# VinAIResearch/GaPro

Measured on AMD Instinct MI355X. Metric: scenes/sec pseudo-label gen (ScanNetV2-train-shaped synthetic scenes), higher is better.
Workload: dtype f64

## Files before the change

### gapro_amd/csrc/svgp_fit.hip

```cpp
#include <math.h>

#include <algorithm>
#include <type_traits>
#include <vector>

#include "common.h"
#include "fit_layout.h"
#include "fit_math.h"
#include "epilogue.h"
#ifdef GAPRO_DEBUG_TU
#include "../../include/gapro_hip_debug.h"
#include "mfma64.h"
#endif

namespace {
using namespace gapro_fit;

#ifndef GAPRO_NT
#define GAPRO_NT 512
#endif
constexpr int NT = GAPRO_NT;
constexpr int NW = NT / 64;
constexpr int kMaxMpLds = 512;
constexpr int kMaxDynLds = 150 * 1024;
// ... 353 lines not shown
                                     const gd* __restrict__ Q, int ld, const gd* __restrict__ qscale, KRange kr,
                                     Epi epi, ldsd* ring) {
  static_assert(NT == 512 || !sizeof(Epi), "gemm_wg: eight waves, one k row of a chunk per wave");
  static_assert(PF == 2 || PF == 4, "gemm_wg: register stages");
  rows16 = uni(rows16);
  cols16 = uni(cols16);
  lower_only = uni((int)lower_only) != 0;
  ld = uni(ld);
  P = uni_ptr(P);
  Q = uni_ptr(Q);
  qscale = uni_ptr(qscale);
  const int wave = uni(threadIdx.x >> 6), lane = threadIdx.x & 63, lr = lane & 15, lq = lane >> 4;
  const int rows = 16 * rows16, cols = 16 * cols16;
  const int nti = (rows + kWgTile - 1) / kWgTile, ntj = (cols + kWgTile - 1) / kWgTile;
  const int wi = wave < 4 ? wave : 7 - wave, wj = wave >> 2;
  const int kmax = TRIM ? uni((g_sh.f.M + 7) / 8 * 8) : ld;
  const int lcol = 2 * lane;
  const int lds_wr = wave * kWgRow + lcol;
  const int fa = lq * kWgRow + 32 * wi + lr;
  const int fb = kWgKC * kWgRow + lq * kWgRow + 64 * wj + lr;
#pragma nounroll
  for (int ti = 0; ti < nti; ++ti) {
#pragma nounroll
    for (int tj = 0; tj < (lower_only ? ti + 1 : ntj); ++tj) {
      const int I0 = kWgTile * ti, J0 = kWgTile * tj;
      int klo = 1 << 30, khi = 0, plo = 1 << 30, phi = 0;
      unsigned on_mask = 0;
      if (rows - I0 >= kWgTile && cols - J0 >= kWgTile) {
        int lo, hi, d;
        kr(I0, J0, &lo, &d);
        kr(I0 + kWgTile - 16, J0 + kWgTile - 16, &d, &hi);
        hi = hi < kmax ? hi : kmax;
        if (lo < hi) { klo = lo; khi = hi; }
        const int pi0 = I0 + 32 * wi, pj0 = J0 + 64 * wj;
#pragma unroll
        for (int u = 0; u < 2; ++u)
#pragma unroll
          for (int v = 0; v < 4; ++v)
            if (!(lower_only && pi0 + 16 * u < pj0 + 16 * v)) on_mask |= 1u << (4 * u + v);
        if (on_mask) {
          kr(pi0, pj0, &lo, &d);
          kr(pi0 + 16, pj0 + 48, &d, &hi);
          hi = hi < kmax ? hi : kmax;
          if (lo < hi) { plo = lo; phi = hi; }
        }
      } else {
#pragma nounroll
        for (int bi = 0; bi < kWgTile / 16; ++bi) {
          const int ib = I0 + 16 * bi;
          if (ib >= rows) break;
#pragma nounroll
          for (int bj = 0; bj < kWgTile / 16; ++bj) {
            const int jb = J0 + 16 * bj;
            if (jb >= cols) break;
            if (lower_only && ib < jb) continue;
            const bool mine = (bi >> 1) == wi && (bj >> 2) == wj;
            if (mine) on_mask |= 1u << (4 * (bi & 1) + (bj & 3));
            int lo, hi;
            kr(ib, jb, &lo, &hi);
            hi = hi < kmax ? hi : kmax;
            if (lo >= hi) continue;
            klo = lo < klo ? lo : klo;
            khi = hi > khi ? hi : khi;
            if (mine) {
              plo = lo < plo ? lo : plo;
              phi = hi > phi ? hi : phi;
            }
          }
        }
      }
      klo = uni(klo) & ~(kWgKC - 1);
      khi = uni(khi);
      plo = uni(plo) & ~(kWgKC - 1);
      phi = uni(phi);
      on_mask = (unsigned)uni((int)on_mask);
      const int nch = klo < khi ? (khi - klo + kWgKC - 1) / kWgKC : 0;
      d4 acc[2][4];
#pragma unroll
      for (int u = 0; u < 2; ++u)
#pragma unroll
        for (int v = 0; v < 4; ++v) acc[u][v] = (d4){0.0, 0.0, 0.0, 0.0};
      if (nch > 0) {
        const bool pin = I0 + lcol < ld, qin = J0 + lcol < ld;
        const gd* pg = P + (size_t)wave * ld + (pin ? I0 + lcol : 0);
        const gd* qg = Q + (size_t)wave * ld + (qin ? J0 + lcol : 0);
        d2 rp[PF], rq[PF];
        double rs[PF];
        auto gload = [&](int n, d2& p, d2& q, double& sc) {
          n = n < nch ? n : nch - 1;
          const size_t o = (size_t)(klo + kWgKC * n) * ld;
          p = *(const g_d2*)(pg + o);
          q = *(const g_d2*)(qg + o);
          if (SCALE) sc = qscale[klo + kWgKC * n + wave];
        };
        auto lstore = [&](int stage, const d2& p, const d2& q, double sc) {
          ldsd* base = ring + stage * kWgStage + lds_wr;
          *(lds_d2*)base = p;
          *(lds_d2*)(base + kWgKC * kWgRow) = SCALE ? (d2){q[0] * sc, q[1] * sc} : q;
        };
        double fa0[2], fb0[4], fa1[2], fb1[4];
        auto rd = [&](int stage, int s, double (&a)[2], double (&b)[4]) {
          const ldsd* st = ring + stage * kWgStage + 4 * s * kWgRow;
#pragma unroll
          for (int v = 0; v < 4; ++v) b[v] = st[fb + 16 * v];
#pragma unroll
          for (int u = 0; u < 2; ++u) a[u] = st[fa + 16 * u];
        };
        auto mm = [&](int k0, const double (&a)[2], const double (&b)[4]) {
          if (k0 < plo || k0 >= phi) return;
#pragma unroll
          for (int u = 0; u < 2; ++u)
#pragma unroll
            for (int v = 0; v < 4; ++v)
              acc[u][v] = __builtin_amdgcn_mfma_f64_16x16x4f64(a[u], b[v], acc[u][v], 0, 0, 0);
        };
        auto chunk = [&](auto cur_tag, auto slot_tag, int c) {
          constexpr int CUR = decltype(cur_tag)::value, SLOT = decltype(slot_tag)::value;
          const int k0 = klo + kWgKC * c;
          lstore(CUR ^ 1, rp[SLOT], rq[SLOT], rs[SLOT]);
          gload(c + 1 + PF, rp[SLOT], rq[SLOT], rs[SLOT]);
          rd(CUR, 1, fa1, fb1);
          __builtin_amdgcn_sched_barrier(0);
          mm(k0, fa0, fb0);
          __builtin_amdgcn_sched_barrier(0);
          __syncthreads();
          rd(CUR ^ 1, 0, fa0, fb0);
          __builtin_amdgcn_sched_barrier(0);
          mm(k0, fa1, fb1);
          __builtin_amdgcn_sched_barrier(0);
        };
        using I0t = std::integral_constant<int, 0>;
        using I1t = std::integral_constant<int, 1>;
        using I2t = std::integral_constant<int, 2>;
        using I3t = std::integral_constant<int, 3>;
#pragma unroll
        for (int n = 0; n < PF; ++n) gload(n, rp[n], rq[n], rs[n]);
        lstore(0, rp[0], rq[0], rs[0]);
        gload(PF, rp[0], rq[0], rs[0]);
        __syncthreads();
        rd(0, 0, fa0, fb0);
        int c = 0;
        if constexpr (PF == 2) {
#pragma nounroll
          for (; c + 1 < nch; c += 2) {
            chunk(I0t{}, I1t{}, c);
            chunk(I1t{}, I0t{}, c + 1);
          }
          if (c < nch) chunk(I0t{}, I1t{}, c);
        } else {
#pragma nounroll
          for (; c + 3 < nch; c += 4) {
            chunk(I0t{}, I1t{}, c);
            chunk(I1t{}, I2t{}, c + 1);
            chunk(I0t{}, I3t{}, c + 2);
            chunk(I1t{}, I0t{}, c + 3);
          }
          if (c < nch) chunk(I0t{}, I1t{}, c);
          if (c + 1 < nch) chunk(I1t{}, I2t{}, c + 1);
          if (c + 2 < nch) chunk(I0t{}, I3t{}, c + 2);
        }
      }
      run_epilogue<8>(epi,
                      [&](int b, int* i, int* j) {
                        const bool on = (on_mask >> b) & 1u;
                        *i = on ? I0 + 32 * wi + 16 * (b >> 2) : -1;
                        *j = J0 + 64 * wj + 16 * (b & 3);
                      },
                      [&](int b) -> const d4& { return acc[b >> 2][b & 3]; });
    }
  }
}

__device__ inline void store_tile(const d4& v, gd* __restrict__ Cm, gd* __restrict__ CT, int ld, int i0, int j0,
                                  ldsd* tile ) {
  const int lane = threadIdx.x & 63, lr = lane & 15, lq = lane >> 4;
  if (Cm) {
#pragma unroll
    for (int r = 0; r < 4; ++r) Cm[(size_t)(i0 + lq + 4 * r) * ld + j0 + lr] = v[r];
  }
  if (CT) {
#pragma unroll
    for (int r = 0; r < 4; ++r) tile[(lq + 4 * r) * 17 + lr] = v[r];
    __builtin_amdgcn_fence(__ATOMIC_RELEASE, "wavefront", "local");
    __builtin_amdgcn_wave_barrier();
#pragma unroll
    for (int r = 0; r < 4; ++r) CT[(size_t)(j0 + lq + 4 * r) * ld + i0 + lr] = tile[lr * 17 + lq + 4 * r];
    __builtin_amdgcn_fence(__ATOMIC_ACQUIRE, "wavefront", "local");
    __builtin_amdgcn_wave_barrier();
  }
}

__device__ __noinline__ void diag_factor_invert(ldsd* panel, int kb) {
  const Fit& f = g_sh.f;
  const int Mp = f.Mp;
  kb = uni(kb);
  gd* LT = f.mat[B_LT];
  const int lane = threadIdx.x & 63, r = lane & 15;
#ifdef GAPRO_PROFILE
  const unsigned long long tp0 = wall_clock64();
#endif
  double rdiag[16];
  {
    double a[16];
#pragma unroll
    for (int c = 0; c < 16; ++c) a[c] = panel[r * 17 + c];
    bool bad = false;
#pragma unroll
    for (int j = 0; j < 16; ++j) {
      double d = lane_bcast(a[j], j);
      if (!(d > 0.0)) {
        bad = true;
        d = 1e-30;
      }
      const double rs = rsqrt(d);
      rdiag[j] = rs;
      const double lj = (r == j) ? d * rs : a[j] * rs;
      a[j] = lj;
#pragma unroll
      for (int c = j + 1; c < 16; ++c) a[c] -= lj * lane_bcast(lj, c);
    }
    if (bad && lane == 0) g_sh.chol_bad = 1;
    if (lane < 16) {
#pragma unroll
      for (int c = 0; c < 16; ++c) g_sh.dblk[r * 17 + c] = (c <= r) ? a[c] : 0.0;
    }
  }
  __builtin_amdgcn_fence(__ATOMIC_SEQ_CST, "wavefront", "local");
  __builtin_amdgcn_wave_barrier();
#ifdef GAPRO_PROFILE
  const unsigned long long tp1 = wall_clock64();
#endif
  {
    double x[16], b[16];
#pragma unroll
    for (int rr = 0; rr < 16; ++rr) b[rr] = (rr == r) ? 1.0 : 0.0;
#pragma unroll
    for (int q = 0; q < 16; ++q) {
      x[q] = (q >= r) ? b[q] * rdiag[q] : 0.0;
#pragma unroll
      for (int rr = q + 1; rr < 16; ++rr) b[rr] = fma(-g_sh.dblk[rr * 17 + q], x[q], b[rr]);
    }
    if (lane < 16) {
#pragma unroll
      for (int c = 0; c < 16; ++c) g_sh.dinv[c * 17 + r] = x[c];
    }
  }
  __builtin_amdgcn_fence(__ATOMIC_SEQ_CST, "wavefront", "local");
  __builtin_amdgcn_wave_barrier();
#ifdef GAPRO_PROFILE
  const unsigned long long tp2 = wall_clock64();
#endif
#pragma unroll
  for (int e = 0; e < 4; ++e) {
    const int idx = lane + 64 * e;
    const int rr = idx >> 4, cc = idx & 15;
    LT[(size_t)(16 * kb + rr) * Mp + 16 * kb + cc] = g_sh.dblk[cc * 17 + rr];
    f.dinv[(size_t)kb * 256 + idx] = g_sh.dinv[rr * 17 + cc];
    f.dinvT[(size_t)kb * 256 + idx] = g_sh.dinv[cc * 17 + rr];
  }
#ifdef GAPRO_PROFILE
  if (lane == 0) {
    const unsigned long long tp3 = wall_clock64();
    g_sh.prof[22] += tp1 - tp0;
    g_sh.prof[23] += tp2 - tp1;
    g_sh.prof[24] += tp3 - tp2;
  }
#endif
}

__device__ inline void chol_update_tile(d4& acc, const gd* pa, const gd* pb, int Mp, int Q) {
  const size_t st = (size_t)4 * Mp;
  auto ld = [&](int q, double (&a)[4], double (&b)[4]) {
    const size_t o = (size_t)q * Mp;
#pragma unroll
    for (int e = 0; e < 4; ++e) {
      a[e] = pa[o + e * st];
      b[e] = pb[o + e * st];
    }
  };
  auto mm = [&](double (&a)[4], double (&b)[4]) {
#pragma unroll
    for (int e = 0; e < 4; ++e) acc = __builtin_amdgcn_mfma_f64_16x16x4f64(-a[e], b[e], acc, 0, 0, 0);
  };
  if (Q <= 0) return;
  double a0[4], b0[4], a1[4], b1[4];
  ld(0, a0, b0);
  int q = 0;
#pragma nounroll
  for (; q + 32 < Q; q += 32) {
    ld(q + 16, a1, b1);
    mm(a0, b0);
    ld(q + 32, a0, b0);
    mm(a1, b1);
  }
  if (q + 16 < Q) {
    ld(q + 16, a1, b1);
    mm(a0, b0);
    mm(a1, b1);
  } else {
    mm(a0, b0);
  }
}

template <int DC>
__device__ __noinline__ void cholesky_fused(const ldsd* Zt, ldsd* panel, double s, double inv_l2, double jitter) {
  const Fit& f = g_sh.f;
  Shared& sh = g_sh;
  const int Mp = f.Mp, M = f.M, D = DC ? DC : f.D, nb = Mp / 16;
  gd* LT = f.mat[B_LT];
  const int wave = __builtin_amdgcn_readfirstlane(threadIdx.x >> 6), lane = threadIdx.x & 63;
  const int lr = lane & 15, lq = lane >> 4;
  for (int kb = 0; kb < nb; ++kb) {
    for (int ib = kb + wave; ib < nb; ib += NW) {
      d4 acc;
      const int col = 16 * kb + lr;
#pragma unroll
      for (int r = 0; r < 4; ++r) {
        const int row = 16 * ib + lq + 4 * r;
        double v = 0.0;
        if (row < M && col < M) {
          v = s * gapro_fit_math::rbf_exp(-0.5 * inv_l2 * sqdist_t(Zt, row, Zt, col, D, Mp));
          if (row == col) v += jitter;
        } else if (row == col) {
          v = 1.0;
        }
        acc[r] = v;
      }
      const gd* pa = LT + (size_t)lq * Mp + 16 * ib + lr;
      const gd* pb = LT + (size_t)lq * Mp + 16 * kb + lr;
      chol_update_tile(acc, pa, pb, Mp, 16 * kb);
      ldsd* dst = panel + (16 * (ib - kb)) * 17;
#pragma unroll
      for (int r = 0; r < 4; ++r) dst[(lq + 4 * r) * 17 + lr] = acc[r];
    }
    __syncthreads();
    prof_stamp(0);
    if (wave == 0) diag_factor_invert(panel, kb);
    __syncthreads();
    prof_stamp(5);
    const int rows_below = Mp - 16 * (kb + 1);
    ldsd* pb = panel + 16 * 17;
    for (int idx = threadIdx.x; idx < rows_below * 16; idx += NT) {
      const int i = idx >> 4, c = idx & 15;
      double acc = 0.0;
#pragma unroll
      for (int q = 0; q < 16; ++q) acc += (q <= c) ? pb[i * 17 + q] * sh.dinv[c * 17 + q] : 0.0;
      __builtin_amdgcn_fence(__ATOMIC_SEQ_CST, "wavefront", "local");
      __builtin_amdgcn_wave_barrier();
      pb[i * 17 + c] = acc;
    }
    __syncthreads();
    if (rows_below > 0)
      for (int idx = threadIdx.x; idx < rows_below * 16; idx += NT) {
        const int c = idx / rows_below, i = idx - c * rows_below;
        LT[(size_t)(16 * kb + c) * Mp + 16 * (kb + 1) + i] = pb[i * 17 + c];
      }
    __syncthreads();
    prof_stamp(18);
  }
}

inline __host__ __device__ int chol_panel_doubles(int Mp) { return Mp * 17 + 64 * 17; }
template <int DC>
__device__ __noinline__ void cholesky_fused_lookahead(const ldsd* Zt, ldsd* panels, double s, double inv_l2,
                                                      double jitter) {
  const Fit& f = g_sh.f;
  Shared& sh = g_sh;
  const int Mp = f.Mp, M = f.M, D = DC ? DC : f.D, nb = Mp / 16;
  gd* LT = f.mat[B_LT];
  const int wave = __builtin_amdgcn_readfirstlane(threadIdx.x >> 6), lane = threadIdx.x & 63;
  const int lr = lane & 15, lq = lane >> 4;
  const int PS = chol_panel_doubles(Mp);
  auto build = [&](int ib, int kb, int qb, ldsd* dst_panel) {
    d4 acc;
    const int col = 16 * kb + lr;
#pragma unroll
    for (int r = 0; r < 4; ++r) {
      const int row = 16 * ib + lq + 4 * r;
      double v = 0.0;
      if (row < M && col < M) {
        v = s * gapro_fit_math::rbf_exp(-0.5 * inv_l2 * sqdist_t(Zt, row, Zt, col, D, Mp));
        if (row == col) v += jitter;
      } else if (row == col) {
        v = 1.0;
      }
      acc[r] = v;
    }
    const gd* pa = LT + (size_t)lq * Mp + 16 * ib + lr;
    const gd* pb = LT + (size_t)lq * Mp + 16 * kb + lr;
    chol_update_tile(acc, pa, pb, Mp, 16 * qb);
    ldsd* dst = dst_panel + (16 * (ib - kb)) * 17;
#pragma unroll
    for (int r = 0; r < 4; ++r) dst[(lq + 4 * r) * 17 + lr] = acc[r];
  };
  for (int ib = wave; ib < nb; ib += NW) build(ib, 0, 0, panels);
  __syncthreads();
  for (int kb = 0; kb < nb; ++kb) {
    ldsd* cur = panels + (kb & 1) * PS;
    ldsd* nxt = panels + ((kb + 1) & 1) * PS;
    if (wave == 0) {
      if (NW <= 4) __builtin_amdgcn_s_setprio(3);
      diag_factor_invert(cur, kb);
      if (NW <= 4) __builtin_amdgcn_s_setprio(0);
    } else {
      for (int ib = kb + wave; ib < nb; ib += NW - 1) build(ib, kb + 1, kb, nxt);
    }
    __syncthreads();
    prof_stamp(5);
    const int rows_below = Mp - 16 * (kb + 1);
    ldsd* pb = cur + 16 * 17;
    for (int idx = threadIdx.x; idx < rows_below * 16; idx += NT) {
      const int i = idx >> 4, c = idx & 15;
      double acc = 0.0;
#pragma unroll
      for (int q = 0; q < 16; ++q) acc += (q <= c) ? pb[i * 17 + q] * sh.dinv[c * 17 + q] : 0.0;
      __builtin_amdgcn_fence(__ATOMIC_SEQ_CST, "wavefront", "local");
      __builtin_amdgcn_wave_barrier();
      pb[i * 17 + c] = acc;
    }
    __syncthreads();
    for (int ib = kb + 1 + wave; ib < nb; ib += NW) {
      ldsd* dst = nxt + (16 * (ib - kb - 1)) * 17;
      const ldsd* la = pb + (16 * (ib - kb - 1) + lr) * 17 + lq;
      const ldsd* lb = pb + lr * 17 + lq;
      d4 acc;
#pragma unroll
      for (int r = 0; r < 4; ++r) acc[r] = dst[(lq + 4 * r) * 17 + lr];
#pragma unroll
      for (int st = 0; st < 4; ++st) acc = __builtin_amdgcn_mfma_f64_16x16x4f64(-la[4 * st], lb[4 * st], acc, 0, 0, 0);
#pragma unroll
      for (int r = 0; r < 4; ++r) dst[(lq + 4 * r) * 17 + lr] = acc[r];
    }
    if (rows_below > 0)
      for (int idx = threadIdx.x; idx < rows_below * 16; idx += NT) {
        const int c = idx / rows_below, i = idx - c * rows_below;
        LT[(size_t)(16 * kb + c) * Mp + 16 * (kb + 1) + i] = pb[i * 17 + c];
      }
    __syncthreads();
    prof_stamp(18);
  }
}

template <int DC, int TMAX>
__device__ __noinline__ void cholesky_fused_lookahead_reg(const ldsd* Zt, ldsd* panel, double s, double inv_l2,
                                                          double jitter) {
  const Fit& f = g_sh.f;
  Shared& sh = g_sh;
  const int Mp = f.Mp, M = f.M, D = DC ? DC : f.D, nb = Mp / 16;
  gd* LT = f.mat[B_LT];
  const int wave = __builtin_amdgcn_readfirstlane(threadIdx.x >> 6), lane = threadIdx.x & 63;
  const int lr = lane & 15, lq = lane >> 4;
  auto build = [&](int ib, int kb, int qb) -> d4 {
    d4 acc;
    const int col = 16 * kb + lr;
#pragma unroll
    for (int r = 0; r < 4; ++r) {
      const int row = 16 * ib + lq + 4 * r;
      double v = 0.0;
      if (row < M && col < M) {
        v = s * gapro_fit_math::rbf_exp(-0.5 * inv_l2 * sqdist_t(Zt, row, Zt, col, D, Mp));
        if (row == col) v += jitter;
      } else if (row == col) {
        v = 1.0;
      }
      acc[r] = v;
    }
    const gd* pa = LT + (size_t)lq * Mp + 16 * ib + lr;
    const gd* pb = LT + (size_t)lq * Mp + 16 * kb + lr;
    chol_update_tile(acc, pa, pb, Mp, 16 * qb);
    return acc;
  };
  for (int ib = wave; ib < nb; ib += NW) {
    const d4 acc = build(ib, 0, 0);
    ldsd* dst = panel + (16 * ib) * 17;
#pragma unroll
    for (int r = 0; r < 4; ++r) dst[(lq + 4 * r) * 17 + lr] = acc[r];
  }
  __syncthreads();
  d4 nx[TMAX];
  for (int kb = 0; kb < nb; ++kb) {
    if (wave == 0) {
      diag_factor_invert(panel, kb);
    } else {
#pragma unroll
      for (int t = 0; t < TMAX; ++t) {
        const int ib = kb + wave + t * (NW - 1);
        if (ib < nb) nx[t] = build(ib, kb + 1, kb);
      }
    }
    __syncthreads();
    prof_stamp(5);
    const int rows_below = Mp - 16 * (kb + 1);
    ldsd* pb = panel + 16 * 17;
    for (int idx = threadIdx.x; idx < rows_below * 16; idx += NT) {
      const int i = idx >> 4, c = idx & 15;
      double acc = 0.0;
#pragma unroll
      for (int q = 0; q < 16; ++q) acc += (q <= c) ? pb[i * 17 + q] * sh.dinv[c * 17 + q] : 0.0;
      __builtin_amdgcn_fence(__ATOMIC_SEQ_CST, "wavefront", "local");
      __builtin_amdgcn_wave_barrier();
      pb[i * 17 + c] = acc;
    }
    __syncthreads();
    if (wave != 0) {
#pragma unroll
      for (int t = 0; t < TMAX; ++t) {
        const int ib = kb + wave + t * (NW - 1);
        if (ib < nb) {
          const ldsd* la = pb + (16 * (ib - kb - 1) + lr) * 17 + lq;
          const ldsd* lb = pb + lr * 17 + lq;
#pragma unroll
          for (int st = 0; st < 4; ++st)
            nx[t] = __builtin_amdgcn_mfma_f64_16x16x4f64(-la[4 * st], lb[4 * st], nx[t], 0, 0, 0);
        }
      }
    }
    if (rows_below > 0)
      for (int idx = threadIdx.x; idx < rows_below * 16; idx += NT) {
        const int c = idx / rows_below, i = idx - c * rows_below;
        LT[(size_t)(16 * kb + c) * Mp + 16 * (kb + 1) + i] = pb[i * 17 + c];
      }
    __syncthreads();
    if (wave != 0) {
#pragma unroll
      for (int t = 0; t < TMAX; ++t) {
        const int ib = kb + wave + t * (NW - 1);
        if (ib < nb) {
          ldsd* dst = panel + (16 * (ib - kb - 1)) * 17;
#pragma unroll
          for (int r = 0; r < 4; ++r) dst[(lq + 4 * r) * 17 + lr] = nx[t][r];
        }
      }
    }
    __syncthreads();
    prof_stamp(18);
  }
}

template <int DC, int LOOKAHEAD>
__device__ __noinline__ void cholesky_psd_safe(const ldsd* Zt, ldsd* scratch, double s, double inv_l2, double jitter,
                                               int retries, double psd_jitter) {
  double extra = 0.0;
  for (int attempt = 0;; ++attempt) {
    if (LOOKAHEAD == 1) cholesky_fused_lookahead<DC>(Zt, scratch, s, inv_l2, jitter + extra);
    else if (LOOKAHEAD == 2) cholesky_fused_lookahead_reg<DC, 3>(Zt, scratch, s, inv_l2, jitter + extra);
    else if (LOOKAHEAD == 3) cholesky_fused_lookahead_reg<DC, 5>(Zt, scratch, s, inv_l2, jitter + extra);
    else cholesky_fused<DC>(Zt, scratch, s, inv_l2, jitter + extra);
    const int bad = g_sh.chol_bad;
    if (!bad) return;
    __syncthreads();
    if (threadIdx.x == 0) {
      g_sh.chol_bad = 0;
      if (attempt >= retries) g_sh.status = GAPRO_ERR_CHOLESKY;
    }
    __syncthreads();
    if (attempt >= retries) return;
    extra = psd_jitter * pow(10.0, (double)attempt);
  }
}

template <int CNT>
__device__ inline void inv_column(int k, ldsd* tile) {
  const Fit& f = g_sh.f;
  const int Mp = f.Mp;
  const gd* LT = f.mat[B_LT];
  gd* LI = f.mat[B_LI];
  gd* U = f.mat[B_U];
  const int lane = threadIdx.x & 63, lr = lane & 15, lq = lane >> 4;
  constexpr int MAXR = CNT > 1 ? CNT - 1 : 1;
  d4 blk[CNT];
  double A0[MAXR * 4], A1[MAXR * 4], D0[4], D1[4];
  auto ldrow = [&](int ii, double (&A)[MAXR * 4], double (&D)[4]) {
    const int i = k + ii;
#pragma unroll
    for (int jj = 0; jj < MAXR; ++jj)
      if (jj < ii) {
        const gd* pa = LT + (size_t)(16 * (k + jj) + lq) * Mp + 16 * i + lr;
#pragma unroll
        for (int st = 0; st < 4; ++st) A[jj * 4 + st] = pa[(size_t)(4 * st) * Mp];
      }
#pragma unroll
    for (int st = 0; st < 4; ++st) D[st] = f.dinvT[(size_t)i * 256 + (4 * st + lq) * 16 + lr];
  };
  d4 dk;
#pragma unroll
  for (int r = 0; r < 4; ++r) dk[r] = f.dinv[(size_t)k * 256 + (lq + 4 * r) * 16 + lr];
  if (CNT > 1) ldrow(1, A1, D1);
  store_tile(dk, LI, U, Mp, 16 * k, 16 * k, tile);
  blk[0] = dk;
#pragma unroll
  for (int ii = 1; ii < CNT; ++ii) {
    if (ii + 1 < CNT) {
      if ((ii + 1) & 1) ldrow(ii + 1, A1, D1);
      else ldrow(ii + 1, A0, D0);
    }
    d4 acc = (d4){0.0, 0.0, 0.0, 0.0};
#pragma unroll
    for (int jj = 0; jj < MAXR; ++jj)
      if (jj < ii) {
#pragma unroll
        for (int st = 0; st < 4; ++st)
          acc = __builtin_amdgcn_mfma_f64_16x16x4f64((ii & 1) ? A1[jj * 4 + st] : A0[jj * 4 + st], blk[jj][st], acc, 0, 0, 0);
      }
    d4 out = (d4){0.0, 0.0, 0.0, 0.0};
#pragma unroll
    for (int st = 0; st < 4; ++st)
      out = __builtin_amdgcn_mfma_f64_16x16x4f64(-((ii & 1) ? D1[st] : D0[st]), acc[st], out, 0, 0, 0);
    store_tile(out, LI, U, Mp, 16 * (k + ii), 16 * k, tile);
    blk[ii] = out;
  }
}
__device__ __noinline__ void tri_inverse_strip(ldsd* tiles) {
  const int nb = g_sh.f.Mp / 16;
  const int wave = __builtin_amdgcn_readfirstlane(threadIdx.x >> 6);
  ldsd* tile = tiles + wave * 16 * 17;
  for (int k = wave; k < nb; k += NW) {
    switch (nb - k) {
      case 1: inv_column<1>(k, tile); break;
      case 2: inv_column<2>(k, tile); break;
      case 3: inv_column<3>(k, tile); break;
      case 4: inv_column<4>(k, tile); break;
#if GAPRO_NT >= 320
      case 5: inv_column<5>(k, tile); break;
      case 6: inv_column<6>(k, tile); break;
      case 7: inv_column<7>(k, tile); break;
      default: inv_column<8>(k, tile); break;
#else
      default: break;
#endif
    }
  }
}

template <int NBR>
__device__ __noinline__ void tri_inverse(ldsd* tiles) {
  const Fit& f = g_sh.f;
  const int Mp = f.Mp, nb = Mp / 16;
  const gd* LT = f.mat[B_LT];
  gd* LI = f.mat[B_LI];
  gd* U = f.mat[B_U];
  const int wave = __builtin_amdgcn_readfirstlane(threadIdx.x >> 6), lane = threadIdx.x & 63;
  const int lr = lane & 15, lq = lane >> 4;
  ldsd* tile = tiles + wave * 16 * 17;
  unsigned long long mine = 0;
  if (NBR == 0) {
    int load[NW];
#pragma unroll
    for (int w = 0; w < NW; ++w) load[w] = 0;
    for (int k = 0; k < nb; ++k) {
      int best = 0;
#pragma unroll
      for (int w = 1; w < NW; ++w) best = load[w] < load[best] ? w : best;
      const int n = nb - k;
#pragma unroll
      for (int w = 0; w < NW; ++w) load[w] += (w == best) ? n * (n - 1) / 2 + 1 : 0;
      if (best == wave) mine |= 1ull << k;
    }
  }
  for (int k = NBR > 0 ? wave : 0; k < nb; k += NBR > 0 ? NW : 1) {
    if (NBR == 0 && !((mine >> k) & 1ull)) continue;
    d4 blk[NBR > 0 ? NBR : 1];
    d4 dk;
#pragma unroll
    for (int r = 0; r < 4; ++r) dk[r] = f.dinv[(size_t)k * 256 + (lq + 4 * r) * 16 + lr];
    store_tile(dk, LI, U, Mp, 16 * k, 16 * k, tile);
    if (NBR > 0) blk[0] = dk;
    if (NBR > 0) {
#pragma unroll
      for (int ii = 1; ii < NBR; ++ii) {
        const int i = k + ii;
        if (i < nb) {
          d4 acc = (d4){0.0, 0.0, 0.0, 0.0};
#pragma unroll
          for (int jj = 0; jj < ii; ++jj) {
            const gd* pa = LT + (size_t)(16 * (k + jj) + lq) * Mp + 16 * i + lr;
#pragma unroll
            for (int sstep = 0; sstep < 4; ++sstep)
              acc = __builtin_amdgcn_mfma_f64_16x16x4f64(pa[(size_t)(4 * sstep) * Mp], blk[jj][sstep], acc, 0, 0, 0);
          }
          d4 out = (d4){0.0, 0.0, 0.0, 0.0};
#pragma unroll
          for (int sstep = 0; sstep < 4; ++sstep) {
            const double a = -f.dinvT[(size_t)i * 256 + (4 * sstep + lq) * 16 + lr];
            out = __builtin_amdgcn_mfma_f64_16x16x4f64(a, acc[sstep], out, 0, 0, 0);
          }
          store_tile(out, LI, U, Mp, 16 * i, 16 * k, tile);
          blk[ii] = out;
        }
      }
    } else {
      for (int i = k + 1; i < nb; ++i) {
        d4 nacc = (d4){0.0, 0.0, 0.0, 0.0};
        __builtin_amdgcn_fence(__ATOMIC_SEQ_CST, "workgroup");
        chol_update_tile(nacc, LT + (size_t)(16 * k + lq) * Mp + 16 * i + lr, LI + (size_t)(16 * k + lq) * Mp + 16 * k + lr,
                         Mp, 16 * (i - k));
        d4 out = (d4){0.0, 0.0, 0.0, 0.0};
#pragma unroll
        for (int sstep = 0; sstep < 4; ++sstep) {
          const double a = f.dinvT[(size_t)i * 256 + (4 * sstep + lq) * 16 + lr];
          out = __builtin_amdgcn_mfma_f64_16x16x4f64(a, nacc[sstep], out, 0, 0, 0);
        }
        store_tile(out, LI, U, Mp, 16 * i, 16 * k, tile);
      }
    }
  }
}

struct ColMap {
  int G, col, grp;
  bool active;
};
__device__ inline ColMap col_map(int Mp) {
  ColMap c;
  c.G = NT / Mp;
  c.col = threadIdx.x % Mp;
  c.grp = threadIdx.x / Mp;
  c.active = c.grp < c.G;
  return c;
}

template <int DC>
__device__ __noinline__ void build_kx(const ldsd* Zt, const ldsd* Pt, int ncols, double s, double inv_l2) {
  const Fit& f = g_sh.f;
  const int Mp = f.Mp, M = f.M, D = DC ? DC : f.D;
  gd* KX = f.mat[B_KX];
  const ColMap cm = col_map(Mp);
  if (!cm.active) return;
  const int n = cm.col;
  for (int k = cm.grp; k < Mp; k += cm.G) {
    double v = 0.0;
    if (k < M && n < ncols) v = s * gapro_fit_math::rbf_exp(-0.5 * inv_l2 * sqdist_t(Zt, k, Pt, n, D, Mp));
    KX[(size_t)k * Mp + n] = v;
  }
}

__device__ __noinline__ void mean_var(double s, double jitter, ldsd* red) {
  const Fit& f = g_sh.f;
  const int Mp = f.Mp;
  const gd* A = f.mat[B_A];
  const gd* BM = f.mat[B_BM];
  const gd* m = f.vec[V_M];
  const ColMap cm = col_map(Mp);
  double pm = 0.0, pv = 0.0;
  if (cm.active) {
    for (int i = cm.grp; i < Mp; i += cm.G) {
      const double a = A[(size_t)i * Mp + cm.col], b = BM[(size_t)i * Mp + cm.col];
      pm += m[i] * a;
      pv += b * b - a * a;
    }
  }
  red[threadIdx.x] = pm;
  red[NT + threadIdx.x] = pv;
  __syncthreads();
  if (threadIdx.x < Mp) {
    double sm = 0.0, sv = 0.0;
    for (int g = 0; g < cm.G; ++g) {
      sm += red[g * Mp + threadIdx.x];
      sv += red[NT + g * Mp + threadIdx.x];
    }
    f.vec[V_MU][threadIdx.x] = sm;
    f.vec[V_VAR][threadIdx.x] = s + jitter + sv;
  }
  __syncthreads();
}

__device__ __noinline__ void weighted_colsum(const gd* Mtx, const gd* w, int Mp, gd* out, ldsd* red) {
  const ColMap cm = col_map(Mp);
  double p = 0.0;
  if (cm.active)
    for (int r = cm.grp; r < Mp; r += cm.G) p += w[r] * Mtx[(size_t)r * Mp + cm.col];
  red[threadIdx.x] = p;
  __syncthreads();
  if (threadIdx.x < Mp) {
    double sacc = 0.0;
    for (int g = 0; g < cm.G; ++g) sacc += red[g * Mp + threadIdx.x];
    out[threadIdx.x] = sacc;
  }
  __syncthreads();
}

__device__ __noinline__ double quadrature(double c, double min_variance, double Nd, bool want_e, ldsd* red,
                                          double* g_c, double* gv_sum) {
  const Fit& f = g_sh.f;
  const int Mp = f.Mp, M = f.M;
  gd* gmu = f.vec[V_GMU];
  gd* gv = f.vec[V_GV];
  double e_tot = 0.0, gc_part = 0.0, gvs_part = 0.0;
  constexpr int PPR = NT / 10;
  const int q = threadIdx.x % 10, nl = threadIdx.x / 10;
  for (int n0 = 0; n0 < M; n0 += PPR) {
    const int n = n0 + nl;
    double E = 0.0, dmu = 0.0, dvar = 0.0;
    const bool on = nl < PPR && n < M;
    if (on) {
      const double mu = f.vec[V_MU][n] + c;
      const double vraw = f.vec[V_VAR][n];
      const double var = vraw < min_variance ? min_variance : vraw;
      const double sd = sqrt(2.0 * var);
      const double y = n < f.M1 ? -1.0 : 1.0;
      const double t = c_gh_t[q], w = c_gh_w[q];
      gh_pair(y, mu, sd, t, w, want_e, &E, &dmu, &dvar);
    }
    red[threadIdx.x] = E;
    red[NT + threadIdx.x] = dmu;
    red[2 * NT + threadIdx.x] = dvar;
    __syncthreads();
    if (on && q == 0) {
      double se = 0.0, sm = 0.0, sv = 0.0;
      for (int qq = 0; qq < 10; ++qq) {
        se += red[threadIdx.x + qq];
        sm += red[NT + threadIdx.x + qq];
        sv += red[2 * NT + threadIdx.x + qq];
      }
      const double ipi = 0.56418958354775628695;
      const double vraw = f.vec[V_VAR][n];
      const bool clamped = vraw < min_variance;
      const double var = clamped ? min_variance : vraw;
      const double y = n < f.M1 ? -1.0 : 1.0;
      const double g1 = -(ipi * sm * y) / Nd;
      const double g2 = clamped ? 0.0 : -(ipi * sv * y / sqrt(2.0 * var)) / Nd;
      gmu[n] = g1;
      gv[n] = g2;
      e_tot += ipi * se;
      gc_part += g1;
      gvs_part += g2;
    }
    __syncthreads();
  }
  for (int n = M + threadIdx.x; n < Mp; n += NT) {
    gmu[n] = 0.0;
    gv[n] = 0.0;
  }
  *g_c = block_sum(gc_part);
  *gv_sum = block_sum(gvs_part);
  return want_e ? block_sum(e_tot) : 0.0;
}

template <int DMAX, bool ZX, int U, int DC>
__device__ __noinline__ void kernel_grads_adam_z(ldsd* Zt, const ldsd* Xt, const gd* Gm, const gd* GTm,
                                                 const gd* GKXT, double s, double inv_l2, double step_size,
                                                 double bc2s, ldsd* red, double* gs_out, double* gl_out,
                                                 const ldsd* zx_rows = nullptr) {
  const Fit& f = g_sh.f;
  const int Mp = f.Mp, M = f.M, D = DC ? DC : f.D;
  const ColMap cm = col_map(Mp);
  const int j = cm.col;
  double acc[DMAX];
#pragma unroll
  for (int d = 0; d < DMAX; ++d) acc[d] = 0.0;
  double gs = 0.0, gl = 0.0;
  if (DMAX > 8) {
    double wsum = 0.0;
    if (cm.active && j < M) {
      for (int i = cm.grp; i < M; i += cm.G) {
        const size_t o = (size_t)i * Mp + j;
        const double gsym = 0.5 * (Gm[o] + GTm[o]);
        const double g3 = ZX ? GKXT[o] : 0.0;
        double d2 = 0.0, d2x = 0.0;
#pragma unroll 8
        for (int d = 0; d < D; ++d) {
          const double zjd = Zt[d * Mp + j];
          const double a = zjd - Zt[d * Mp + i];
          d2 += a * a;
          if (ZX) {
            const double bx = zjd - Xt[d * Mp + i];
            d2x += bx * bx;
          }
        }
        const double e = gapro_fit_math::rbf_exp(-0.5 * inv_l2 * d2);
        const double w = gsym * s * e;
        gs += gsym * e;
        gl += w * d2;
        double wx = 0.0;
        if (ZX) {
          const double ex = gapro_fit_math::rbf_exp(-0.5 * inv_l2 * d2x);
          wx = g3 * s * ex;
          gs += g3 * ex;
          gl += wx * d2x;
        }
        wsum += 2.0 * w + wx;
#pragma unroll
        for (int d = 0; d < DMAX; ++d)
          if (d < D) acc[d] += 2.0 * w * Zt[d * Mp + i] + (ZX ? wx * Xt[d * Mp + i] : 0.0);
      }
    }
#pragma unroll
    for (int d = 0; d < DMAX; ++d) acc[d] = (d < D) ? wsum * Zt[d * Mp + j] - acc[d] : 0.0;
  } else if (cm.active && j < M) {
    double zj[DMAX];
#pragma unroll
    for (int d = 0; d < DMAX; ++d) zj[d] = (d < D) ? Zt[d * Mp + j] : 0.0;
    for (int i0 = cm.grp; i0 < M; i0 += cm.G * U) {
      double g1[U], g2[U], g3[U];
#pragma unroll
      for (int u = 0; u < U; ++u) {
        const int i = i0 + u * cm.G;
        const bool act = i < M;
        const size_t o = (size_t)(act ? i : 0) * Mp + j;
        g1[u] = act ? Gm[o] : 0.0;
        g2[u] = act ? GTm[o] : 0.0;
        g3[u] = (ZX && act) ? GKXT[o] : 0.0;
      }
#pragma unroll
      for (int u = 0; u < U; ++u) {
        const int i = i0 + u * cm.G;
        if (u * cm.G >= M) break;
        if (i < M) {
          double t[DMAX];
          double d2 = 0.0;
#pragma unroll
          for (int d = 0; d < DMAX; ++d) {
            t[d] = (d < D) ? zj[d] - Zt[d * Mp + i] : 0.0;
            d2 += t[d] * t[d];
          }
          const double e = gapro_fit_math::rbf_exp(-0.5 * inv_l2 * d2);
          const double gsym = 0.5 * (g1[u] + g2[u]);
          const double w = gsym * s * e;
          gs += gsym * e;
          gl += w * d2;
#pragma unroll
          for (int d = 0; d < DMAX; ++d) acc[d] += 2.0 * w * t[d];
          if (ZX) {
            double d2x = 0.0;
#pragma unroll
            for (int d = 0; d < DMAX; ++d) {
              t[d] = (d < D) ? zj[d] - Xt[d * Mp + i] : 0.0;
              d2x += t[d] * t[d];
            }
            const double ex = gapro_fit_math::rbf_exp(-0.5 * inv_l2 * d2x);
            const double wx = g3[u] * s * ex;
            gs += g3[u] * ex;
            gl += wx * d2x;
#pragma unroll
            for (int d = 0; d < DMAX; ++d) acc[d] += wx * t[d];
          }
        }
      }
    }
  }
  prof_stamp(20);
  *gs_out = block_sum(gs);
  *gl_out = block_sum(gl);
  prof_stamp(21);
  const double b1 = 0.9, b2 = 0.999, aeps = 1e-8;
#pragma unroll
  for (int dc = 0; dc < DMAX; dc += kRedSlots) {
    if (dc < D) {
#pragma unroll
      for (int e = 0; e < kRedSlots; ++e)
        if (dc + e < DMAX) red[e * NT + threadIdx.x] = acc[dc + e];
      __syncthreads();
      if (threadIdx.x < M) {
#pragma unroll
        for (int e = 0; e < kRedSlots; ++e) {
          const int d = dc + e;
          if (d < D && d < DMAX) {
            double sacc = 0.0;
            for (int g = 0; g < cm.G; ++g) sacc += red[e * NT + g * Mp + threadIdx.x];
            const size_t zi = (size_t)threadIdx.x * D + d;
            if (!ZX) sacc += zx_rows ? zx_rows[threadIdx.x * 8 + d] : f.gZ[zi];
            const double grad = -inv_l2 * sacc;
            f.gZ[zi] = grad;
            const double m1 = b1 * f.mZ[zi] + (1.0 - b1) * grad;
            const double m2 = b2 * f.vZ[zi] + (1.0 - b2) * grad * grad;
            f.mZ[zi] = m1;
            f.vZ[zi] = m2;
            const double znew = f.Z[zi] - step_size * m1 / (sqrt(m2) / bc2s + aeps);
            f.Z[zi] = znew;
            Zt[d * Mp + threadIdx.x] = znew;
          }
        }
      }
      __syncthreads();
    }
  }
}

template <int WG, int TU, bool SCALE, int ORD, int PK = 0, int QK = 0, typename KRange, typename Epi>
__device__ inline void product(int mo, int no, bool lower, const gd* __restrict__ P, const gd* __restrict__ Q, int ld,
                               const gd* __restrict__ qs, KRange kr, Epi epi, ldsd* ring) {
  if constexpr (WG == 0) {
    gemm_tn_in<TU, SCALE, 2, ORD, true, PK, QK>(mo, no, lower, P, Q, ld, qs, kr, epi);
  } else {
    const int rows = (16 * mo + 31) / 32 * 32, cols = (16 * no + 31) / 32 * 32;
    const int R = rows / kWgTile * kWgTile, Cc = cols / kWgTile * kWgTile;
    constexpr bool kMajor = !(PK || QK);
    if constexpr (kMajor) {
      if (R > 0 && Cc > 0 && !lower) gemm_wg<SCALE, true, WG>(R / 16, Cc / 16, false, P, Q, ld, qs, kr, epi, ring);
    }
    auto strip_t = [&](auto tu_tag, int r0, int c0, int nr, int nc, bool low) {
      constexpr int TUS = decltype(tu_tag)::value;
      if (nr <= 0 || nc <= 0) return;
      gemm_tn_in<TUS, SCALE, 2, ORD_ROWMAJOR, true, PK, QK>(
          nr / (8 * TUS), nc / (8 * TUS), low, PK ? P + (size_t)r0 * ld : P + r0, QK ? Q + (size_t)c0 * ld : Q + c0, ld, qs,
          [=](int i0, int j0, int* lo, int* hi) {
            int l0, h0, l1, h1;
            kr(r0 + i0, c0 + j0, &l0, &h0);
            kr(r0 + i0 + 16 * TUS - 16, c0 + j0 + 16 * TUS - 16, &l1, &h1);
            *lo = l0;
            *hi = h1;
          },
          shifted_epi(epi, r0, c0));
    };
    auto strip = [&](int r0, int c0, int nr, int nc, bool low) {
      strip_t(std::integral_constant<int, 2>{}, r0, c0, nr, nc, low);
    };
    if (lower) {
      if constexpr (WG == 4) {
        if (rows >= 352) {
          strip_t(std::integral_constant<int, 4>{}, 0, 0, rows, cols, true);
          return;
        }
      }
      strip(0, 0, rows, cols, true);
      return;
    }
    if constexpr (kMajor) {
      strip(R, 0, rows - R, cols, false);
      strip(0, Cc, R, cols - Cc, false);
    } else {
      strip(0, 0, rows, cols, false);
    }
  }
}

template <int TU, int DMAX, int DC, int WG = 0, bool KMIN = false, int EG = 4>
__device__ void fit_body(const gapro_fit_options& opt, ldsd* Zt, ldsd* Pt, ldsd* scratch, const gapro_fit_desc& desc, float* __restrict__ o_probs, float* __restrict__ o_probs_new,
                         unsigned char* __restrict__ o_labels, float* __restrict__ o_mu, float* __restrict__ o_var,
                         double* loss_out) {
  const Fit& f = g_sh.f;
  Shared& sh = g_sh;
  const int M = f.M, Mp = f.Mp, D = DC ? DC : f.D, T = f.T;
  constexpr int TS = 16 * TU;
  constexpr int TSB = TU >= 2 ? 8 * TU : TS;
  const int mt = Mp / TSB;
  const double Nd = (double)M;
  const double jitter = opt.jitter;
  gd* LS = f.mat[B_LS];
  gd* LST = f.mat[B_LST];
  gd* MLS = f.mat[B_MLS];
  gd* VLS = f.mat[B_VLS];
  gd* A = f.mat[B_A];
  gd* AT = KMIN ? nullptr : f.mat[B_AT];
  gd* BM = f.mat[B_BM];
  gd* BMT = f.mat[B_BMT];
  gd* GA = f.mat[B_GA];
  gd* GKXT = f.mat[B_GKXT];
  gd* GAT = KMIN ? nullptr : GKXT;
  gd* vm = f.vec[V_M];
  gd* gmu = f.vec[V_GMU];
  gd* gv = f.vec[V_GV];
  ldsd* ring = scratch;
  ldsd* tile = scratch + (WG ? kWgStage : 0) + (threadIdx.x >> 6) * 16 * 17;
  static_assert(WG == 0 || TU == 1, "workgroup-tiled products take their extents and ranges per 16 x 16 block");
  double last_loss = 0.0;
#ifdef GAPRO_PROFILE
  auto stamp = [&](int id) {
    __syncthreads();
    if (threadIdx.x == 0) {
      const unsigned long long t = wall_clock64();
      sh.prof[id] += t - sh.t_last;
      sh.t_last = t;
    }
  };
#else
  auto stamp = [&](int) {};
#endif
#if defined(GAPRO_PROFILE) && defined(GAPRO_PROFILE_SPLIT)
#define STAMP_MERGED(id) do { __syncthreads(); stamp(id); } while (0)
#else
#define STAMP_MERGED(id) do { if constexpr (!KMIN) __syncthreads(); } while (0)
#endif

  auto refresh_hypers = [&]() {
    __syncthreads();
    if (threadIdx.x == 0) {
      sh.s = softplus(sh.rho_s);
      sh.ell = softplus(sh.rho_l);
      sh.inv_l2 = 1.0 / (sh.ell * sh.ell);
    }
    __syncthreads();
  };
  auto factorize = [&]() {
    stamp(19);
    cholesky_psd_safe<DC, KMIN ? 0 : 3>(Zt, scratch, sh.s, sh.inv_l2, jitter, opt.psd_retries, opt.psd_jitter);
    stamp(1);
    if (Mp <= 128)
      tri_inverse<8>(scratch);
    else
      tri_inverse<0>(scratch);
    __syncthreads();
    stamp(2);
  };
  const bool fuse = Mp <= kFuseMaxMp;
  ldsd* part_m = scratch + kTileDoubles;
  ldsd* part_a = part_m + (Mp / 16) * Mp;
  ldsd* part_b = part_a + (Mp / 16) * Mp;
  gd* gpart_m = f.mat[B_GA];
  gd* gpart_a = gpart_m + (size_t)(Mp / 16) * Mp;
  gd* gpart_b = gpart_a + (size_t)(Mp / 16) * Mp;
  auto forward_products = [&](int ncols, double s_, double jitter_) {
    const int nt = (ncols + TSB - 1) / TSB;
    product<WG, TU, false, ORD_ROWS_DESC>(mt, nt, false, f.mat[B_U], f.mat[B_KX], Mp, nullptr,
                       [=](int i0, int, int* lo, int* hi) { *lo = 0; *hi = i0 + TS; },
                       [=](int i, int n, const d4& v) {
                         if constexpr (KMIN) store_tile(v, A, nullptr, Mp, i, n, tile);
                         else store_tile(v, A, AT, Mp, i, n, tile);
                         {
                           const int lane = threadIdx.x & 63, lr = lane & 15, lq = lane >> 4;
                           double pm = 0.0, pa = 0.0;
#pragma unroll
                           for (int r = 0; r < 4; ++r) {
                             pm += vm[i + lq + 4 * r] * v[r];
                             pa += v[r] * v[r];
                           }
                           pm += __shfl_xor(pm, 16, 64);
                           pa += __shfl_xor(pa, 16, 64);
                           pm += __shfl_xor(pm, 32, 64);
                           pa += __shfl_xor(pa, 32, 64);
                           if (lq == 0) {
                             if (fuse) {
                               part_m[(i >> 4) * Mp + n + lr] = pm;
                               part_a[(i >> 4) * Mp + n + lr] = pa;
                             } else {
                               gpart_m[(size_t)(i >> 4) * Mp + n + lr] = pm;
                               gpart_a[(size_t)(i >> 4) * Mp + n + lr] = pa;
                             }
                           }
                         }
                       }, ring);
    __syncthreads();
    if constexpr (KMIN) {
    product<WG, TU, false, ORD_ROWMAJOR>(mt, nt, false, LS, A, Mp, nullptr,
                       [=](int j0, int, int* lo, int* hi) { *lo = j0; *hi = Mp; },
                       [=](int j, int n, const d4& v) {
                         store_tile(v, BM, nullptr, Mp, j, n, tile);
                         {
                           const int lane = threadIdx.x & 63, lr = lane & 15, lq = lane >> 4;
                           double pb = 0.0;
#pragma unroll
                           for (int r = 0; r < 4; ++r) pb += v[r] * v[r];
                           pb += __shfl_xor(pb, 16, 64);
                           pb += __shfl_xor(pb, 32, 64);
                           if (lq == 0) {
                             if (fuse) part_b[(j >> 4) * Mp + n + lr] = pb;
                             else gpart_b[(size_t)(j >> 4) * Mp + n + lr] = pb;
                           }
                         }
                       }, ring);
    } else {
    product<WG, TU, false, ORD_COLMAJOR>(nt, mt, false, A, LS, Mp, nullptr,
                       [=](int, int j0, int* lo, int* hi) { *lo = j0; *hi = Mp; },
                       [=](int n, int j, const d4& v) {
                         store_tile(v, BMT, BM, Mp, n, j, tile);
                         {
                           const int lane = threadIdx.x & 63, lr = lane & 15, lq = lane >> 4;
#pragma unroll
                           for (int r = 0; r < 4; ++r) {
                             double pb = v[r] * v[r];
                             pb += __shfl_xor(pb, 1, 64);
                             pb += __shfl_xor(pb, 2, 64);
                             pb += __shfl_xor(pb, 4, 64);
                             pb += __shfl_xor(pb, 8, 64);
                             if (lr == 0) {
                               if (fuse) part_b[(j >> 4) * Mp + n + lq + 4 * r] = pb;
                               else gpart_b[(size_t)(j >> 4) * Mp + n + lq + 4 * r] = pb;
                             }
                           }
                         }
                       }, ring);
    }
    __syncthreads();
    for (int n = threadIdx.x; n < nt * TSB; n += NT) {
      double sm = 0.0, sa = 0.0, sb = 0.0;
      if (fuse) {
        for (int tq = 0; tq < Mp / 16; ++tq) {
          sm += part_m[tq * Mp + n];
          sa += part_a[tq * Mp + n];
          sb += part_b[tq * Mp + n];
        }
      } else {
        for (int tq = 0; tq < Mp / 16; ++tq) {
          sm += gpart_m[(size_t)tq * Mp + n];
          sa += gpart_a[(size_t)tq * Mp + n];
          sb += gpart_b[(size_t)tq * Mp + n];
        }
      }
      f.vec[V_MU][n] = sm;
      f.vec[V_VAR][n] = s_ + jitter_ + (sb - sa);
    }
    __syncthreads();
  };

  auto step_fn = [&](int step) __attribute__((noinline)) {
    refresh_hypers();
    const double s = sh.s, ell = sh.ell, inv_l2 = sh.inv_l2, c = sh.c;
    const bool last = step == opt.training_iter;
    factorize();
    build_kx<DC>(Zt, Pt, M, s, inv_l2);
    __syncthreads();
    stamp(3);
    forward_products(M, s, jitter);
    stamp(4);
    double g_c, gv_sum;
    const double e_sum = quadrature(c, opt.min_variance, Nd, last, scratch, &g_c, &gv_sum);
    if (last) {
      double kl_part = 0.0;
      for (int idx = threadIdx.x; idx < M * M; idx += NT) {
        const int i = idx / M, j = idx - i * M;
        if (j <= i) {
          const double v = LS[(size_t)i * Mp + j];
          kl_part += v * v;
          if (i == j) kl_part -= log(v * v);
        }
      }
      for (int i = threadIdx.x; i < M; i += NT) kl_part += vm[i] * vm[i];
      const double kl = 0.5 * (block_sum(kl_part) - Nd);
      last_loss = -(e_sum / Nd - kl / Nd);
    }
    stamp(6);

    const double b1 = 0.9, b2 = 0.999, aeps = 1e-8;
    const double bc1 = 1.0 - pow(b1, (double)step), bc2s = sqrt(1.0 - pow(b2, (double)step));
    const double step_size = opt.lr / bc1;
    gd* gpart_g = f.mat[B_GKX];
    struct GaPre { double a[4], m[4], gvn, gmn; };
    product<WG, TU, false, ORD_ROWS_DESC>(mt, mt, false, LST, BM, Mp, nullptr,
                       [=](int i0, int, int* lo, int* hi) { *lo = 0; *hi = i0 + TS; },
                       two_phase_epi<EG>(
                       [=](int i0, int n0) {
                         const int lane = threadIdx.x & 63, lr = lane & 15, lq = lane >> 4;
                         const int n = n0 + lr;
                         GaPre p;
                         p.gvn = gv[n];
                         p.gmn = gmu[n];
#pragma unroll
                         for (int r = 0; r < 4; ++r) {
                           const int i = i0 + lq + 4 * r;
                           p.a[r] = A[(size_t)i * Mp + n];
                           p.m[r] = vm[i];
                         }
                         return p;
                       },
                       [=](int i0, int n0, const d4& v, const GaPre& p) {
                         const int lane = threadIdx.x & 63, lr = lane & 15, lq = lane >> 4;
                         const int n = n0 + lr;
                         const double gvn = p.gvn, gmn = p.gmn;
                         d4 ga;
#pragma unroll
                         for (int r = 0; r < 4; ++r) {
                           const int i = i0 + lq + 4 * r;
                           const double a = p.a[r];
                           ga[r] = 2.0 * gvn * v[r] + p.m[r] * gmn - 2.0 * a * gvn;
                           if constexpr (KMIN) GA[(size_t)i * Mp + n] = ga[r];
                           double pg = a * gmn;
                           pg += __shfl_xor(pg, 1, 64);
                           pg += __shfl_xor(pg, 2, 64);
                           pg += __shfl_xor(pg, 4, 64);
                           pg += __shfl_xor(pg, 8, 64);
                           if (lr == 0) {
                             if (fuse) part_m[(n0 >> 4) * Mp + i] = pg;
                             else gpart_g[(size_t)(n0 >> 4) * Mp + i] = pg;
                           }
                         }
                         if constexpr (!KMIN) store_tile(ga, GA, GAT, Mp, i0, n0, tile);
                       }), ring);
    __syncthreads();
    for (int i = threadIdx.x; i < Mp; i += NT) {
      double sg = 0.0;
      if (fuse) {
        for (int tq = 0; tq < Mp / 16; ++tq) sg += part_m[tq * Mp + i];
      } else {
        for (int tq = 0; tq < Mp / 16; ++tq) sg += gpart_g[(size_t)tq * Mp + i];
      }
      f.vec[V_GM][i] = sg;
    }
    __syncthreads();
    stamp(7);
    struct LsPre { double l[4], m1[4], m2[4]; };
    auto gls_epi = two_phase_epi<EG>(
                      [=](int i0, int j0) {
                        const int lane = threadIdx.x & 63, lr = lane & 15, lq = lane >> 4;
                        const int j = j0 + lr;
                        LsPre p;
#pragma unroll
                        for (int r = 0; r < 4; ++r) {
                          const size_t o = (size_t)(i0 + lq + 4 * r) * Mp + j;
                          p.l[r] = LS[o];
                          p.m1[r] = MLS[o];
                          p.m2[r] = VLS[o];
                        }
                        return p;
                      },
                      [=](int i0, int j0, const d4& v, const LsPre& p) {
                        const int lane = threadIdx.x & 63, lr = lane & 15, lq = lane >> 4;
                        const int j = j0 + lr;
                        d4 newv;
#pragma unroll
                        for (int r = 0; r < 4; ++r) {
                          const int i = i0 + lq + 4 * r;
                          const size_t o = (size_t)i * Mp + j;
                          double lnew = 0.0;
                          if (j <= i && i < M) {
                            const double l = p.l[r];
                            const double g = 2.0 * v[r] + (l - (i == j ? 1.0 / l : 0.0)) / Nd;
                            const double m1 = b1 * p.m1[r] + (1.0 - b1) * g;
                            const double m2 = b2 * p.m2[r] + (1.0 - b2) * g * g;
                            MLS[o] = m1;
                            VLS[o] = m2;
                            lnew = l - step_size * m1 / (sqrt(m2) / bc2s + aeps);
                            LS[o] = lnew;
                          }
                          newv[r] = lnew;
                        }
                        store_tile(newv, nullptr, LST, Mp, i0, j0, tile);
                      });
    auto gls_range = [=](int, int, int* lo, int* hi) { *lo = 0; *hi = Mp; };
    if constexpr (KMIN)
      product<WG, TU, true, ORD_ROWMAJOR, 1, 1>(mt, mt, true, A, BM, Mp, gv, gls_range, gls_epi, ring);
    else
      product<WG, TU, true, ORD_ROWMAJOR>(mt, mt, true, AT, BMT, Mp, gv, gls_range, gls_epi, ring);
    STAMP_MERGED(8);
    gd* Pm = f.mat[B_L];
    auto pm_range = [=](int, int, int* lo, int* hi) { *lo = 0; *hi = Mp; };
    if constexpr (KMIN) {
      product<WG, TU, false, ORD_ROWMAJOR, 1, 1>(mt, mt, true, GA, A, Mp, nullptr, pm_range,
                       [=](int i0, int j0, const d4& v) {
                         const int lane = threadIdx.x & 63, lr = lane & 15, lq = lane >> 4;
#pragma unroll
                         for (int r = 0; r < 4; ++r) {
                           const int i = i0 + lq + 4 * r, j = j0 + lr;
                           Pm[(size_t)i * Mp + j] = (j < i) ? -v[r] : (j == i ? -0.5 * v[r] : 0.0);
                         }
                       }, ring);
    } else {
      product<WG, TU, false, ORD_ROWMAJOR>(mt, mt, true, GAT, AT, Mp, nullptr, pm_range,
                       [=](int i0, int j0, const d4& v) {
                         const int lane = threadIdx.x & 63, lr = lane & 15, lq = lane >> 4;
                         d4 pv;
#pragma unroll
                         for (int r = 0; r < 4; ++r) {
                           const int i = i0 + lq + 4 * r, j = j0 + lr;
                           pv[r] = (j < i) ? -v[r] : (j == i ? -0.5 * v[r] : 0.0);
                         }
                         store_tile(pv, nullptr, Pm, Mp, i0, j0, tile);
                       }, ring);
    }
    STAMP_MERGED(9);
    product<WG, TU, false, ORD_COLMAJOR>(mt, mt, false, GA, f.mat[B_LI], Mp, nullptr,
                       [=](int, int i0, int* lo, int* hi) { *lo = i0; *hi = Mp; },
                       [=](int n, int i, const d4& v) { store_tile(v, GKXT, nullptr, Mp, n, i, tile); }, ring);
    __syncthreads();
    stamp(10);
    stamp(11);
    gd* Wm = f.mat[B_GLS];
    auto w_epi = [=](int i0, int j0, const d4& v) {
                         const int lane = threadIdx.x & 63, lr = lane & 15, lq = lane >> 4;
#pragma unroll
                         for (int r = 0; r < 4; ++r) {
                           const int i = i0 + lq + 4 * r, j = j0 + lr;
                           Wm[(size_t)i * Mp + j] = (j <= i) ? v[r] : 0.0;
                         }
                       };
    auto w_range = [=](int i0, int j0, int* lo, int* hi) { *lo = j0; *hi = i0 + TS; };
    if constexpr (KMIN)
      product<WG, TU, false, ORD_ROWMAJOR, 1, 0>(mt, mt, true, Pm, f.mat[B_LI], Mp, nullptr, w_range, w_epi, ring);
    else
      product<WG, TU, false, ORD_ROWMAJOR>(mt, mt, true, Pm, f.mat[B_LI], Mp, nullptr, w_range, w_epi, ring);
    __syncthreads();
    stamp(12);
    gd* G = BM;
    gd* GT = A;
    product<WG, TU, false, ORD_SHELLS>(mt, mt, false, f.mat[B_LI], Wm, Mp, nullptr,
                       [=](int i0, int j0, int* lo, int* hi) { *lo = i0 > j0 ? i0 : j0; *hi = Mp; },
                       [=](int i, int j, const d4& v) { store_tile(v, G, GT, Mp, i, j, tile); }, ring);
    __syncthreads();
    stamp(13);
    double g_s, g_l;
    kernel_grads_adam_z<DMAX, true, (DMAX <= 8 ? 2 : 1), DC>(Zt, Pt, G, GT, GKXT, s, inv_l2, step_size, bc2s, scratch, &g_s,
                                                         &g_l);
    g_s += gv_sum;
    g_l /= (ell * ell * ell);
    stamp(14);

    auto adam_upd = [&](double p, double& m1, double& m2, double g) {
      m1 = b1 * m1 + (1.0 - b1) * g;
      m2 = b2 * m2 + (1.0 - b2) * g * g;
      return p - step_size * m1 / (sqrt(m2) / bc2s + aeps);
    };
    for (int i = threadIdx.x; i < M; i += NT) {
      const double g = f.vec[V_GM][i] + vm[i] / Nd;
      f.vec[V_GM][i] = g;
      double m1 = f.vec[V_MM][i], m2 = f.vec[V_VM][i];
// ... 1627 lines not shown
```

Baseline: 381.0.

## Interleave triangular inverse rows into Cholesky panel loop with load-balanced tiles

Computes each completed block row of the inverse Cholesky factor inside the blocked Cholesky loop, one step behind the current panel. Tiles are assigned to waves by a greedy least-loaded scheduler that takes each wave's lookahead work into account, and only the last row is finished afterwards in a tail pass. This is meant to hide the separate triangular-inverse phase behind the factorization's idle waves. It relies on dinv/dinvT and LI being ready in global memory at the right step, and the non-KMIN path now depends on the fused Cholesky variant being used.

```diff
diff --git a/gapro_amd/csrc/svgp_fit.hip b/gapro_amd/csrc/svgp_fit.hip
--- a/gapro_amd/csrc/svgp_fit.hip
+++ b/gapro_amd/csrc/svgp_fit.hip
@@ -679,6 +679,69 @@
   }
 }
 
+__device__ inline void inv_tile(int i, int k) {
+  const Fit& f = g_sh.f;
+  const int Mp = f.Mp;
+  const gd* LT = f.mat[B_LT];
+  gd* LI = f.mat[B_LI];
+  gd* U = f.mat[B_U];
+  const int lane = threadIdx.x & 63, lr = lane & 15, lq = lane >> 4;
+  d4 out;
+  if (i == k) {
+#pragma unroll
+    for (int r = 0; r < 4; ++r) out[r] = f.dinv[(size_t)k * 256 + (lq + 4 * r) * 16 + lr];
+  } else {
+    d4 nacc = (d4){0.0, 0.0, 0.0, 0.0};
+    chol_update_tile(nacc, LT + (size_t)(16 * k + lq) * Mp + 16 * i + lr, LI + (size_t)(16 * k + lq) * Mp + 16 * k + lr,
+                     Mp, 16 * (i - k));
+    out = (d4){0.0, 0.0, 0.0, 0.0};
+#pragma unroll
+    for (int st = 0; st < 4; ++st) {
+      const double a = f.dinvT[(size_t)i * 256 + (4 * st + lq) * 16 + lr];
+      out = __builtin_amdgcn_mfma_f64_16x16x4f64(a, nacc[st], out, 0, 0, 0);
+    }
+  }
+#pragma unroll
+  for (int r = 0; r < 4; ++r) {
+    LI[(size_t)(16 * i + lq + 4 * r) * Mp + 16 * k + lr] = out[r];
+    U[(size_t)(16 * k + lr) * Mp + 16 * i + lq + 4 * r] = out[r];
+  }
+}
+__device__ inline int least_loaded(const int (&load)[NW]) {
+  int best = 0, bl = load[0];
+#pragma unroll
+  for (int w = 1; w < NW; ++w)
+    if (load[w] < bl) {
+      bl = load[w];
+      best = w;
+    }
+  return best;
+}
+__device__ inline void inv_row(int r, int (&load)[NW]) {
+  const int wave = __builtin_amdgcn_readfirstlane(threadIdx.x >> 6);
+  for (int k = 0; k <= r; ++k) {
+    const int best = least_loaded(load);
+#pragma unroll
+    for (int w = 0; w < NW; ++w) load[w] += (w == best) ? r - k + 1 : 0;
+    if (best == wave) inv_tile(r, k);
+  }
+}
+constexpr int kDiagLoad = 4;
+__device__ inline void lookahead_loads(int kb, int nb, int (&load)[NW]) {
+  load[0] = kDiagLoad;
+#pragma unroll
+  for (int w = 1; w < NW; ++w) {
+    const int first = kb + w;
+    load[w] = first < nb ? ((nb - 1 - first) / (NW - 1) + 1) * (kb + 1) : 0;
+  }
+}
+__device__ __noinline__ void tri_inverse_tail() {
+  int load[NW];
+#pragma unroll
+  for (int w = 0; w < NW; ++w) load[w] = 0;
+  inv_row(g_sh.f.Mp / 16 - 1, load);
+}
+
 template <int DC>
 __device__ __noinline__ void cholesky_fused(const ldsd* Zt, ldsd* panel, double s, double inv_l2, double jitter) {
   const Fit& f = g_sh.f;
@@ -864,6 +927,11 @@
         const int ib = kb + wave + t * (NW - 1);
         if (ib < nb) nx[t] = build(ib, kb + 1, kb);
       }
+    }
+    if (kb > 0) {
+      int load[NW];
+      lookahead_loads(kb, nb, load);
+      inv_row(kb - 1, load);
     }
     __syncthreads();
     prof_stamp(5);
@@ -1462,10 +1530,14 @@
     stamp(19);
     cholesky_psd_safe<DC, KMIN ? 0 : 3>(Zt, scratch, sh.s, sh.inv_l2, jitter, opt.psd_retries, opt.psd_jitter);
     stamp(1);
-    if (Mp <= 128)
-      tri_inverse<8>(scratch);
-    else
-      tri_inverse<0>(scratch);
+    if constexpr (KMIN) {
+      if (Mp <= 128)
+        tri_inverse<8>(scratch);
+      else
+        tri_inverse<0>(scratch);
+    } else {
+      tri_inverse_tail();
+    }
     __syncthreads();
     stamp(2);
   };
```

After: 383.1 (median of 6 runs). About the same (+0.5%).
